# 0Setsuna0/SoftbodyUnity

Measured on AMD Instinct MI355X. Metric: particle-substeps/sec, higher is better.
Workload: dtype f32

## Files before the change

softbodyunity_amd/csrc/schedule.hip:

```cpp
#include "solver_internal.hpp"
#include "tile_kernel.hip.hpp"
#include "aux_kernels.hip.hpp"

namespace sbi {

sbk::TickParams tick_params(const sb_solver *s, float dt, int substeps) {
    sbk::TickParams t{};
    volatile float S = (float)substeps;
    volatile float h = dt / S;
    t.h = h;
    volatile float inv_h = 1.0f / h;
    t.inv_h = inv_h;
    volatile float hx = h * s->desc.gravity[0], hy = h * s->desc.gravity[1], hz = h * s->desc.gravity[2];
    t.hgx = hx; t.hgy = hy; t.hgz = hz;
    volatile float td = s->desc.damping * h;
    volatile float kd = 1.0f - td;
    t.kd = kd < 0.0f ? 0.0f : (float)kd;
    volatile float h2 = h * h;
    volatile float ad = s->compliance[0] / h2;
    volatile float av = s->compliance[1] / h2;
    volatile float av36 = 36.0f * av;
    volatile float ab = s->compliance[2] / h2;
    t.at_d = ad; t.at_v = av36; t.at_b = ab;
    t.pnx = s->plane[0]; t.pny = s->plane[1]; t.pnz = s->plane[2]; t.pd = s->plane[3]; t.plane_on = s->plane_on;
// ... 112 lines not shown
        int cs = D.send_off[k + 1] - D.send_off[k], cr = D.recv_off[k + 1] - D.recv_off[k];
        if (s->loopback) cs = cr = std::min(cs, cr);
        const size_t fl = with_prev ? 6 : 3;
        if (cs) NCCL_CHECK(rccl().Send(s->d_sendbuf.p + fl * D.send_off[k], fl * (size_t)cs, ncclFloat, s->loopback ? 0 : D.peers[k], s->comm, st));
        if (cr) NCCL_CHECK(rccl().Recv(s->d_recvbuf.p + fl * D.recv_off[k], fl * (size_t)cr, ncclFloat, s->loopback ? 0 : D.peers[k], s->comm, st));
    }
}

void halo_exchange_post(sb_solver *s, int slot, hipStream_t st) {
    if (!halo_slot_active(s, slot) || s->peer.enabled) return;
    DevHalo &D = *s->halos[slot];
    const bool with_prev = slot == 1;
    const int nr = D.recv_off.back();
    if (nr && !(with_prev && s->fused_unpack)) {
        if (with_prev)
            hipLaunchKernelGGL(sbk::halo_unpack_kernel<true>, dim3((nr + 255) / 256), dim3(256), 0, st, s->pos_view(),
                               s->d_prev.p, D.recv_idx.p, s->d_recvbuf.p, nr);
        else
            hipLaunchKernelGGL(sbk::halo_unpack_kernel<false>, dim3((nr + 255) / 256), dim3(256), 0, st, s->pos_view(),
                               s->d_prev.p, D.recv_idx.p, s->d_recvbuf.p, nr);
    }
}

void ExchangeTimer::mark(hipStream_t st, bool join) {
    Event e;
    if (free_list.empty()) e.create(); else { e = std::move(free_list.back()); free_list.pop_back(); }
    HIP_CHECK(hipEventRecord(e, st));
    (join ? join_pending : pending).push_back(std::move(e));
}
void ExchangeTimer::recycle() {
    for (auto *v : {&pending, &join_pending}) {
        free_list.insert(free_list.end(), std::make_move_iterator(v->begin()), std::make_move_iterator(v->end()));
        v->clear();
    }
}

void halo_exchange(sb_solver *s, int slot, hipStream_t st) {
    if (!st) st = s->stream;
    if (!halo_slot_active(s, slot)) return;
    const bool timed = s->xtimer.enabled && !s->capturing;
    if (timed) s->xtimer.mark(st);
    if (!s->peer.enabled) halo_exchange_pre(s, slot, st);
    if (timed) s->xtimer.mark(st);
    if (s->peer.enabled) halo_exchange_pre(s, slot, st);
    if (!s->peer.enabled) {
        NCCL_CHECK(rccl().GroupStart());
        try {
            halo_exchange_calls(s, slot, st);
        } catch (...) {
            (void)rccl().GroupEnd();
            throw;
        }
        NCCL_CHECK(rccl().GroupEnd());
    }
    halo_exchange_post(s, slot, st);
    if (timed) s->xtimer.mark(st);
}

template <int KIND>
void launch_tile(sb_solver *s, DevTiling &D, int tile_begin = 0, int tile_end = -1, int halo = sbk::kHaloNone, const sbk::TileDesc *table = nullptr) {
    const bool ghosts = halo == sbk::kHaloGhosts;
    if (tile_end < 0) tile_end = D.n_tiles;
    if (tile_end <= tile_begin) return;
    sbk::TileArgs A{};
    A.pos = s->pos_view(); A.w8 = s->d_w8.p; A.wpal = s->d_wpal.p; A.prev = s->d_prev.p; A.vel = s->d_vel.p;
    A.tiles = D.tiles.p; A.runs_overflow = D.runs_overflow.p; A.stream = D.stream.p;
    A.tp = s->d_tp.p;
    A.gather = D.gather.p;
    A.w_uniform = s->w_uniform ? 1 : 0;
    A.item_waves = D.item_waves;
    A.store_through = tile_end - tile_begin <= s->store_through_max_tiles ? 3 : s->store_through_large;
    A.ghost_src = ghosts ? s->d_recvbuf.p : nullptr; A.n_owned = (int32_t)s->n_owned;
    A.peek_out = KIND == 4 ? s->d_peek.p : nullptr;
    A.kin_map = KIND == 5 ? s->d_kin_map.p : nullptr; A.kin_target = KIND == 5 ? s->d_kin_target.p : nullptr;
    A.max_local = D.max_local; A.win_dwords = D.win_dwords; A.tile_base = tile_begin; A.pal_dwords = D.pal_dwords; A.rounds_dwords = D.rounds_dwords;
    const sbk::TileDesc *tiles_at_base = table ? table : D.tiles.p + tile_begin;
    const int n_wg = tile_end - tile_begin;
    const bool small = D.max_local <= sbk::kSmallTile;
    const bool narrow = small && (D.packed_lanes ? D.packed_lanes == sbk::kLanePackLanes : (s->tile_lanes ? s->tile_lanes == sbk::kNarrowTileThreads : tile_end - tile_begin >= s->narrow_min_tiles));
    const bool quad8 = D.has_quads && s->quad_lanes == sbk::kQuadTileThreads;
    constexpr int kWide8MaxTiles = sbk::kWide8MaxTiles;
    const bool wide8 = small && !D.has_quads && !D.packed_lanes && (s->tile_lanes ? s->tile_lanes == 512 : tile_end - tile_begin <= kWide8MaxTiles);
    const dim3 grid(tile_end - tile_begin), block(quad8 || wide8 ? sbk::kQuadTileThreads : (narrow ? sbk::kNarrowTileThreads : sbk::kWideTileThreads));
#define SB_LAUNCH_TILE(Q, W, G)                                                                                               \
    do {                                                                                                                      \
        if (Q && quad8) {                                                                                                     \
            if (small) hipLaunchKernelGGL((sbk::tile_kernel<KIND, true, sbk::kQuadTileThreads, sbk::kSmallTile / sbk::kQuadTileThreads, W, sbk::kHaloNone>), \
                                          grid, block, D.lds_bytes + s->lds_pad, s->stream, tiles_at_base, n_wg, A);                                           \
            else hipLaunchKernelGGL((sbk::tile_kernel<KIND, true, sbk::kQuadTileThreads, sbk::kLargeTile / sbk::kQuadTileThreads, W, sbk::kHaloNone>), \
                                    grid, block, D.lds_bytes + s->lds_pad, s->stream, tiles_at_base, n_wg, A);                                                 \
        } else if (wide8) hipLaunchKernelGGL((sbk::tile_kernel<KIND, false, sbk::kQuadTileThreads, sbk::kSmallTile / sbk::kQuadTileThreads, W, G>), \
                                       grid, block, D.lds_bytes + s->lds_pad, s->stream, tiles_at_base, n_wg, A);                                              \
        else if (narrow) hipLaunchKernelGGL((sbk::tile_kernel<KIND, Q, sbk::kNarrowTileThreads, sbk::kSmallTile / sbk::kNarrowTileThreads, W, G>), \
                                       grid, block, D.lds_bytes + s->lds_pad, s->stream, tiles_at_base, n_wg, A);                                              \
        else if (small) hipLaunchKernelGGL((sbk::tile_kernel<KIND, Q, sbk::kWideTileThreads, sbk::kSmallTile / sbk::kWideTileThreads, W, G>), \
                                           grid, block, D.lds_bytes + s->lds_pad, s->stream, tiles_at_base, n_wg, A);                                          \
        else hipLaunchKernelGGL((sbk::tile_kernel<KIND, Q, sbk::kWideTileThreads, sbk::kLargeTile / sbk::kWideTileThreads, W, G>), \
                                grid, block, D.lds_bytes + s->lds_pad, s->stream, tiles_at_base, n_wg, A);                                                     \
    } while (0)
    constexpr bool kCanGhost = KIND == 1 || KIND == 2;
    if (ghosts && !(kCanGhost && !D.has_quads)) throw std::runtime_error("internal: ghost-reading tile kernel requested for a launch that has none");
    if (kCanGhost && ghosts) {
        if (s->w_palette) SB_LAUNCH_TILE(false, true, (kCanGhost ? sbk::kHaloGhosts : sbk::kHaloNone)); else SB_LAUNCH_TILE(false, false, (kCanGhost ? sbk::kHaloGhosts : sbk::kHaloNone));
    } else
    if (s->w_palette) { if (D.has_quads) SB_LAUNCH_TILE(true, true, sbk::kHaloNone); else SB_LAUNCH_TILE(false, true, sbk::kHaloNone); }
    else { if (D.has_quads) SB_LAUNCH_TILE(true, false, sbk::kHaloNone); else SB_LAUNCH_TILE(false, false, sbk::kHaloNone); }
#undef SB_LAUNCH_TILE
}

struct LaunchTimer {
    std::vector<Event> ev;
    std::vector<int> slot;
    hipStream_t stream;
    void begin(int which) {
        Event a, b;
        a.create(); b.create();
        HIP_CHECK(hipEventRecord(a, stream));
        ev.push_back(std::move(a)); ev.push_back(std::move(b)); slot.push_back(which);
    }
    void end() { HIP_CHECK(hipEventRecord(ev.back(), stream)); }
};

void launch_tick_kernel(sb_solver *s, int it, int substeps, LaunchTimer *lt, int tile_begin = 0, int tile_end = -1, bool kin = false) {
    const int tl = s->plan->plan.tiling ? (it & 1) : 0;
    DevTiling &D = s->tiling[tl];
    if (lt && D.n_tiles) lt->begin(it == 0 ? 2 + (int)s->gcolours.size() : (it == substeps ? 3 + (int)s->gcolours.size() : tl));
    const int halo_in = s->fused_unpack && tl == 1 ? sbk::kHaloGhosts : sbk::kHaloNone;
    if (it == 0) launch_tile<0>(s, D, tile_begin, tile_end);
    else if (it < substeps && kin) launch_tile<5>(s, D, tile_begin, tile_end);
    else if (it < substeps) launch_tile<1>(s, D, tile_begin, tile_end, halo_in);
    else launch_tile<2>(s, D, tile_begin, tile_end, halo_in);
    if (lt && D.n_tiles) lt->end();
}

void launch_t2_layer(sb_solver *s, int layer, LaunchTimer *lt, bool with_halo = true) {
    const auto rg = s->t2_layer_range[layer];
    if (with_halo) halo_exchange(s, 2 + (int)s->gcolours.size() + layer);
    if (rg.second <= rg.first) return;
    if (lt) lt->begin(4 + (int)s->gcolours.size());
    launch_tile<3>(s, s->tiling[2], rg.first, rg.second);
    if (lt) lt->end();
}

void launch_gcolour(sb_solver *s, int gc, LaunchTimer *lt) {
    DevGColour &G = *s->gcolours[gc];
    if (G.count == 0) return;
    if (lt) lt->begin(2 + gc);
    dim3 grid((G.count + 255) / 256);
    if (G.type == 0)
        hipLaunchKernelGGL(sbk::global_distance_kernel, grid, dim3(256), 0, s->stream, s->pos_view(), G.ij.p, G.rest.p, G.count,
                           s->d_tp.p);
    else
        hipLaunchKernelGGL(sbk::global_quad_kernel, grid, dim3(256), 0, s->stream, s->pos_view(), G.quad.p, G.rest2.p, G.count,
                           G.type, s->d_tp.p);
    if (lt) lt->end();
}

std::vector<TickStep> tick_program(const sb_solver *s, int substeps, bool fused_first, bool defer_last, bool kin) {
    std::vector<TickStep> P;
    const bool two = s->plan->plan.tiling;
    auto tile = [&](int it, TileRange rg, bool k = false) {
        const bool ff = it == 0 && fused_first;
        P.push_back(TickStep{StepKind::Tile, rg, k && ff, ff ? 2 : it, ff ? 4 : substeps, 0});
    };
    if (s->overlap_halo) {
        for (int it = 0; it <= substeps; ++it) {
            if (it == substeps && defer_last) break;
            if (it & 1) {
                tile(it, TileRange::T1Interior);
                P.push_back(TickStep{StepKind::JoinExchange, TileRange::All, false, it, substeps, 1});
                tile(it, TileRange::T1Boundary);
            } else {
                tile(it, TileRange::T0Boundary);
                if (it < substeps) P.push_back(TickStep{StepKind::ForkExchange, TileRange::All, false, it, substeps, 1});
                tile(it, TileRange::T0Interior);
            }
        }
        return P;
    }
    for (int it = 0; it <= substeps; ++it) {
        if (it == substeps && defer_last) break;
        if (two && (it & 1)) P.push_back(TickStep{StepKind::Exchange, TileRange::All, false, it, substeps, 1});
        tile(it, TileRange::All, kin);
        if (it == substeps) break;
        for (size_t ly = 0; ly < s->t2_layer_range.size(); ++ly) {
            P.push_back(TickStep{StepKind::Exchange, TileRange::All, false, it, substeps, 2 + (int)s->gcolours.size() + (int)ly});
            P.push_back(TickStep{StepKind::T2Layer, TileRange::All, false, it, substeps, (int)ly});
        }
        for (size_t gc = 0; gc < s->gcolours.size(); ++gc) {
// ... 404 lines not shown
```

softbodyunity_amd/csrc/tile_kernel.hip.hpp:

```cpp
#pragma once
#include "device_math.hip.hpp"

namespace sbk {

__device__ __forceinline__ void lds_barrier() { asm volatile("s_waitcnt lgkmcnt(0)\n\ts_barrier" ::: "memory"); }

template <bool QUADS, int THREADS> constexpr int kWavesPerSimd = QUADS ? (THREADS == 64 ? 3 : (THREADS == 512 ? 2 : 4)) : (THREADS == 256 ? 8 : (THREADS == 128 ? 6 : 4));
template <int KIND_, bool QUADS, int THREADS, int PPT, bool WPAL, int HALO = kHaloNone>
__global__ __launch_bounds__(THREADS, (kWavesPerSimd<QUADS, THREADS> - (KIND_ == 5 && !QUADS ? 1 : 0))) void tile_kernel(const TileDesc *tiles_at_base, int n_workgroups, TileArgs A) {
    constexpr int KIND = KIND_ == 5 ? 1 : KIND_;
    constexpr bool KIN = KIND_ == 5;
    constexpr bool GHOSTS = HALO == kHaloGhosts;
    constexpr int kTileThreads = THREADS;
    constexpr int kCPL = THREADS >= kRoundSlots ? 1 : kRoundSlots / THREADS;
    extern __shared__ uint4 lds_raw[];
    float4 *lds_pos = reinterpret_cast<float4 *>(lds_raw);
    uint32_t *s_rounds = reinterpret_cast<uint32_t *>(lds_pos + A.max_local);
    float *s_pal = reinterpret_cast<float *>(s_rounds + A.rounds_dwords);
    uint32_t *cbuf = s_rounds + A.rounds_dwords + A.pal_dwords;
    f32x3 *lds_spare = reinterpret_cast<f32x3 *>(cbuf + A.win_dwords);
    typedef const TileDesc __attribute__((address_space(4))) *ConstTileDescPtr;
#ifndef SB_NO_XCD_REMAP
    const int nwg = n_workgroups, wg = (int)blockIdx.x;
    const int xq = nwg >> 3, xr = nwg & 7, xcd = wg & 7;
    const int tile_index = (xcd < xr ? xcd * (xq + 1) : xr * (xq + 1) + (xcd - xr) * xq) + (wg >> 3);
#else
    const int tile_index = (int)blockIdx.x;
#endif
    const TileDesc __attribute__((address_space(4))) &td = *((ConstTileDescPtr)(uintptr_t)tiles_at_base + tile_index);
    const int n_rounds_all = td.n_rounds;
    const int tid = threadIdx.x;
    const int n_local = td.n_local;
    const int run_count = td.run_count;
    const TickParams tp = *A.tp;
    const uint32_t *tstream = A.stream + td.s_begin;
#if defined(SB_ABLATE) && SB_ABLATE == 4
    if (n_local >= 0) { if (n_rounds_all == 0x7fffffff) A.vel[0] = tp.h; return; }
#endif

    int g[PPT];
    if (KIND == 3) {
#pragma unroll
        for (int m = 0; m < PPT; ++m) {
            const int l = tid + m * kTileThreads;
            g[m] = l < n_local ? A.gather[td.gather_begin + l] : -1;
        }
    } else {
        int run_d[kInlineRuns], run_y[kInlineRuns];
#pragma unroll
        for (int r = 0; r < kInlineRuns; ++r) { run_y[r] = td.runs[r].y; run_d[r] = td.runs[r].x - td.runs[r].y; }
#pragma unroll
        for (int m = 0; m < PPT; ++m) {
            const int l = tid + m * kTileThreads;
            int d = run_d[0];
#pragma unroll
            for (int r = 1; r < kInlineRuns; ++r) d = l >= run_y[r] ? run_d[r] : d;
            int gi = l + d;
            if (run_count > kInlineRuns)
                for (int r = kInlineRuns; r < run_count; ++r) {
                    const int2 rn = A.runs_overflow[td.run_overflow + r - kInlineRuns];
                    if (rn.y <= l) gi = rn.x + (l - rn.y);
                }
            g[m] = l < n_local ? gi : -1;
        }
    }
    const int R = n_rounds_all;
    const int v_begin = KIND == 0 ? R : 0;
    const int v_end = KIND == 3 ? R : (KIND == 2 || KIND == 4 ? R + 1 : 2 * R + 1);
    const uint32_t d_lo = td.s_hdr;
    const uint32_t d_hi = td.s_len;
    const uint32_t win = (uint32_t)A.win_dwords;
    uint32_t win_lo = d_lo;
    auto load_window = [&](uint32_t lo) {
        const uint32_t n4 = (min(lo + win, d_hi) - lo) >> 2;
        const uint4 *src = reinterpret_cast<const uint4 *>(tstream + lo);
        uint4 *dst = reinterpret_cast<uint4 *>(cbuf);
        uint32_t t0 = (uint32_t)tid;
        asm volatile("" : "+v"(t0));
        for (uint32_t i = t0; i < n4; i += 4 * kTileThreads) {
            uint4 v0 = src[i], v1, v2, v3;
            const bool b1 = i + kTileThreads < n4, b2 = i + 2 * kTileThreads < n4, b3 = i + 3 * kTileThreads < n4;
            if (b1) v1 = src[i + kTileThreads];
            if (b2) v2 = src[i + 2 * kTileThreads];
            if (b3) v3 = src[i + 3 * kTileThreads];
            dst[i] = v0;
            if (b1) dst[i + kTileThreads] = v1;
            if (b2) dst[i + 2 * kTileThreads] = v2;
            if (b3) dst[i + 3 * kTileThreads] = v3;
        }
    };
    f32x4 X[PPT];
    float pvx[PPT], pvy[PPT], pvz[PPT];
    uint32_t wi[PPT];
    const int mypal = WPAL ? __float_as_int(A.wpal[tid & (kMaxMassPalette - 1)]) : 0;
#pragma unroll
    for (int m = 0; m < PPT; ++m) {
        const int gc = max(g[m], 0);
        const bool ghost = GHOSTS && gc >= A.n_owned;
        const float *px = ghost ? A.ghost_src + 6 * (size_t)(gc - A.n_owned) : A.pos.xyz + 3 * (size_t)gc;
        X[m].x = px[0]; X[m].y = px[1]; X[m].z = px[2];
        if (WPAL) { wi[m] = A.w8[A.w_uniform ? 0 : gc]; X[m].w = 0.0f; } else { wi[m] = 0; X[m].w = A.pos.w[gc]; }
        pvx[m] = pvy[m] = pvz[m] = 0.0f;
        if (KIND != 0 && KIND != 3 && KIND != 4) {
            const float *pp = ghost ? px + 3 : A.prev + 3 * (size_t)gc;
            pvx[m] = pp[0]; pvy[m] = pp[1]; pvz[m] = pp[2];
        }
    }
    const bool rounds_in_lds = n_rounds_all <= A.rounds_dwords;
    const uint32_t rw = tstream[max(min(tid, n_rounds_all - 1), 0)];
    const bool rounds_in_lanes = n_rounds_all <= 64;
    const uint32_t rwl = tstream[max(min(tid & 63, n_rounds_all - 1), 0)];
    uint32_t itreg = 0;
    if (QUADS && kTileThreads == 64 * A.item_waves) {
        const int ns = td.n_steps;
        itreg = tstream[ns > 0 ? td.s_items + (uint32_t)((tid >> 6) * ns + min(tid & 63, ns - 1)) : 0u];
    }
    const int n_pal = td.n_pal;
    const uint32_t palw = tstream[tid < n_pal ? ((n_rounds_all + 3) & ~3) + tid : 0];
#ifndef SB_KW
#define SB_KW (QUADS ? 4 : 2)
#endif
    constexpr int kW = SB_KW;
    const bool lane_packed = !QUADS && kTileThreads == kLanePackLanes && td.packed_lanes == (uint32_t)kLanePackLanes;
    const bool lane_packed_full = !WPAL && lane_packed && td.n_pal == 0;
    const bool wide_packed = !QUADS && kTileThreads == kWidePackLanes && td.packed_lanes == (uint32_t)kWidePackLanes;
    const bool any_packed = lane_packed || wide_packed;
    const uint32_t n4_first = wide_packed ? 0u : lane_packed ? (lane_packed_full ? 2u * (uint32_t)kLanePackLanes : (uint32_t)kLanePackLanes)
                                          : (min(win_lo + win, d_hi) - win_lo) >> 2;
    const u32x4 *wsrc = reinterpret_cast<const u32x4 *>(tstream + win_lo);
    u32x4 wv[kW];
#pragma unroll
    for (int q = 0; q < kW; ++q) {
        const uint32_t i = tid + q * kTileThreads;
        wv[q] = i < n4_first ? wsrc[i] : *reinterpret_cast<const u32x4 *>(tstream);
    }
    typedef uint32_t u32x2 __attribute__((ext_vector_type(2)));
    u32x2 wc = {0u, 0u};
    u32x2 wp = {0u, 0u};
    if (!QUADS && kTileThreads == kWidePackLanes)
        wp = *reinterpret_cast<const u32x2 *>(wide_packed ? tstream + win_lo + 2u * (uint32_t)tid : tstream);
#pragma unroll
    for (int m = 0; m < PPT; ++m) asm volatile("" ::"v"(X[m].x), "v"(pvx[m]), "v"(wi[m]), "v"(X[m].w));
    asm volatile("" ::"v"(mypal));
    if (WPAL) {
#pragma unroll
        for (int m = 0; m < PPT; ++m) X[m].w = __int_as_float(__builtin_amdgcn_ds_bpermute((int)(wi[m] << 2), mypal));
    }
#pragma unroll
    for (int q = 0; q < kW; ++q) asm volatile("" ::"v"(wv[q].x));
    asm volatile("" ::"v"(rw), "v"(palw), "v"(rwl), "v"(itreg));
    if (!QUADS && kTileThreads == kWidePackLanes) asm volatile("" ::"v"(wp.x));
#pragma unroll
    for (int m = 0; m < PPT; ++m)
        if (g[m] >= 0) *reinterpret_cast<f32x4 *>(lds_pos + tid + m * kTileThreads) = X[m];
    if (rounds_in_lds && tid < n_rounds_all) s_rounds[tid] = rw;
    if (tid < n_pal) s_pal[tid] = __uint_as_float(palw);
    if (kTileThreads < kMaxRoundsLds && rounds_in_lds)
        for (int q = tid + kTileThreads; q < n_rounds_all; q += kTileThreads) s_rounds[q] = tstream[q];
    if (kTileThreads < kMaxPalette)
        for (int q = tid + kTileThreads; q < n_pal; q += kTileThreads) s_pal[q] = __uint_as_float(tstream[((n_rounds_all + 3) & ~3) + q]);
    {
        u32x4 *dst = reinterpret_cast<u32x4 *>(cbuf);
#pragma unroll
        for (int q = 0; q < kW; ++q) {
            const uint32_t i = tid + q * kTileThreads;
            if (i < n4_first && !any_packed) dst[i] = wv[q];
        }
        if (!any_packed)
            for (uint32_t i = tid + kW * kTileThreads; i < n4_first; i += kTileThreads) dst[i] = wsrc[i];
    }
    __syncthreads();
    if (!WPAL && !QUADS && kTileThreads == kLanePackLanes && lane_packed_full)
        wc = *reinterpret_cast<const u32x2 *>(tstream + win_lo + 8u * (uint32_t)kLanePackLanes + 2u * (uint32_t)tid);
#if defined(SB_ABLATE) && SB_ABLATE == 5
    if (n_local >= 0) { if (lds_pos[tid].x == 1.2345e-30f && cbuf[tid] == 0x12345678u) A.vel[0] = tp.h; return; }
#endif

    auto mark_step = [&]() {
#pragma unroll
        for (int m = 0; m < PPT; ++m)
            if (g[m] >= 0) {
                const int l = tid + m * kTileThreads;
                float4 P = lds_pos[l];
                if (KIND != 0 && tp.plane_on && P.w > 0.0f) {
                    float a = tp.pnx * P.x, b = tp.pny * P.y, c = tp.pnz * P.z;
                    float pen = ((a + b) + c) - tp.pd;
                    if (pen < 0.0f) {
                        float dx = pen * tp.pnx, dy = pen * tp.pny, dz = pen * tp.pnz;
                        P.x = P.x - dx; P.y = P.y - dy; P.z = P.z - dz;
                        if (KIND == 2 || KIND == 4) lds_pos[l] = P;
                    }
                }
                if (KIND == 4) continue;
                float vx, vy, vz;
                const size_t o = 3 * (size_t)g[m];
                if (KIND == 0) {
                    vx = A.vel[o + 0]; vy = A.vel[o + 1]; vz = A.vel[o + 2];
                } else {
                    float dx = P.x - pvx[m], dy = P.y - pvy[m], dz = P.z - pvz[m];
                    float qx = dx * tp.inv_h, qy = dy * tp.inv_h, qz = dz * tp.inv_h;
                    vx = qx * tp.kd; vy = qy * tp.kd; vz = qz * tp.kd;
                }
                bool moved = false;
                if (KIN && P.w == 0.0f) {
                    const int ks = A.kin_map[g[m]];
                    if (ks >= 0) {
                        float *t = A.kin_target + 3 * (size_t)ks;
                        const float tx = t[0], ty = t[1], tz = t[2];
                        if (tx == tx) { P.x = tx; P.y = ty; P.z = tz; moved = true; t[0] = __int_as_float(0x7fc00000); }
                    }
                }
                if (KIND == 2) {
                    A.vel[o + 0] = vx; A.vel[o + 1] = vy; A.vel[o + 2] = vz;
                } else {
                    if (A.store_through & 1) store3_through(A.prev + o, P.x, P.y, P.z);
                    else { A.prev[o + 0] = P.x; A.prev[o + 1] = P.y; A.prev[o + 2] = P.z; }
                    if (P.w > 0.0f) {
                        vx = vx + tp.hgx; vy = vy + tp.hgy; vz = vz + tp.hgz;
                        float hx = tp.h * vx, hy = tp.h * vy, hz = tp.h * vz;
                        P.x = P.x + hx; P.y = P.y + hy; P.z = P.z + hz;
                        lds_pos[l] = P;
                    } else if (KIN && moved) lds_pos[l] = P;
                }
            }
    };

    constexpr int kRegRounds = THREADS >= 256 ? kRegRoundsWide : kRegRoundsNarrow;
    if (kRegRounds > 0 && !QUADS && n_rounds_all <= kRegRounds && n_rounds_all > 0 && (kRegFullSlots || n_pal > 0) && (any_packed || d_hi - d_lo <= win)) {
        const bool tile_compact = n_pal > 0;
        uint32_t rs[kRegRounds > 0 ? kRegRounds : 1][kCPL];
        float rl[kRegRounds > 0 ? kRegRounds : 1][kCPL];
        int rcnt[kRegRounds > 0 ? kRegRounds : 1];
        {
            uint32_t o = 0;
#pragma unroll
            for (int r = 0; r < kRegRounds; ++r) {
                rcnt[r] = 0;
                if (r < n_rounds_all) {
                    rcnt[r] = (int)((uint32_t)__builtin_amdgcn_readlane((int)rwl, r) & 1023u);
                    if (kCPL == 2 && lane_packed) {
#pragma unroll
                        for (int u = 0; u < kCPL; ++u) {
                            const int bit = kLanePackFieldBits * (2 * r + u), w0 = bit >> 5, sh = bit & 31;
                            const uint32_t lo = wv[0][w0] >> sh;
                            const uint32_t hi = (sh + kLanePackFieldBits > 32) ? (wv[0][w0 + 1 < 4 ? w0 + 1 : 3] << ((32 - sh) & 31)) : 0u;
                            const uint32_t f = (lo | hi) & ((1u << kLanePackFieldBits) - 1u);
                            rs[r][u] = (f & 511u) | (((f >> 9) & 511u) << 12) | ((f >> 18) << 24);
                            if (!WPAL) {
                                const int fld = 2 * r + u;
                                rl[r][u] = __uint_as_float(fld < 4 ? wv[1][fld < 4 ? fld : 0] : wc[fld >= 4 ? fld - 4 : 0]);
                            }
                        }
                    } else if (kCPL == 1 && wide_packed) {
                        const uint64_t two = (uint64_t)wp.x | ((uint64_t)wp.y << 32);
                        const uint32_t f = (uint32_t)(two >> (kLanePackFieldBits * (r < kLanePackRounds ? r : 0))) & ((1u << kLanePackFieldBits) - 1u);
                        rs[r][0] = (f & 511u) | (((f >> 9) & 511u) << 12) | ((f >> 18) << 24);
                    } else if (tile_compact) {
#pragma unroll
                        for (int u = 0; u < kCPL; ++u) {
                            const int c = tid + u * kTileThreads;
                            rs[r][u] = cbuf[o + (c < rcnt[r] ? c : 0)];
                        }
                        o += ((uint32_t)rcnt[r] + 3u) & ~3u;
                    } else {
#pragma unroll
                        for (int u = 0; u < kCPL; ++u) {
                            const int c = tid + u * kTileThreads;
                            const uint2 e = *reinterpret_cast<const uint2 *>(cbuf + o + 2 * (c < rcnt[r] ? c : 0));
                            rs[r][u] = (e.x & 0xfffu) | ((e.x >> 16) << 12);
                            rl[r][u] = __uint_as_float(e.y);
                        }
                        o += (2u * (uint32_t)rcnt[r] + 3u) & ~3u;
                    }
                } else {
#pragma unroll
                    for (int u = 0; u < kCPL; ++u) { rs[r][u] = 0; rl[r][u] = 0.0f; }
                }
            }
            if (tile_compact) {
#pragma unroll
                for (int r = 0; r < kRegRounds; ++r)
#pragma unroll
                    for (int u = 0; u < kCPL; ++u) rl[r][u] = s_pal[rs[r][u] >> 24];
            }
        }
        auto reg_round = [&](const uint32_t (&e)[kCPL], const float (&L0)[kCPL], int cnt) {
            if (kCPL == 1) {
                if (tid < cnt) {
                    const int i = e[0] & 0xfffu, k = (e[0] >> 12) & 0xfffu;
                    float4 a = lds_pos[i], b = lds_pos[k];
                    if (project_distance(a, b, L0[0], tp.at_d)) { lds_pos[i] = a; lds_pos[k] = b; }
                }
            } else {
                int ci[kCPL], ck[kCPL];
                bool con[kCPL];
                f32x4 ca[kCPL], cb[kCPL];
#pragma unroll
                for (int u = 0; u < kCPL; ++u) {
                    con[u] = tid + u * kTileThreads < cnt;
                    ci[u] = e[u] & 0xfffu; ck[u] = (e[u] >> 12) & 0xfffu;
                    ca[u] = *reinterpret_cast<const f32x4 *>(lds_pos + ci[u]);
                    cb[u] = *reinterpret_cast<const f32x4 *>(lds_pos + ck[u]);
                }
#pragma unroll
                for (int u = 0; u < kCPL; ++u) {
                    float4 a = make_float4(ca[u].x, ca[u].y, ca[u].z, ca[u].w), b = make_float4(cb[u].x, cb[u].y, cb[u].z, cb[u].w);
                    con[u] = project_distance_nobranch(a, b, L0[u], tp.at_d) && con[u];
                    ca[u].x = a.x; ca[u].y = a.y; ca[u].z = a.z; cb[u].x = b.x; cb[u].y = b.y; cb[u].z = b.z;
                }
#pragma unroll
                for (int u = 0; u < kCPL; ++u) {
                    f32x3 *da = con[u] ? reinterpret_cast<f32x3 *>(lds_pos + ci[u]) : lds_spare;
                    f32x3 *db = con[u] ? reinterpret_cast<f32x3 *>(lds_pos + ck[u]) : lds_spare;
                    *da = (f32x3){ca[u].x, ca[u].y, ca[u].z};
                    *db = (f32x3){cb[u].x, cb[u].y, cb[u].z};
                }
            }
            lds_barrier();
        };
#if defined(SB_ABLATE) && SB_ABLATE == 1
        constexpr bool kRunRounds = false;
#else
        constexpr bool kRunRounds = true;
#endif
        if (KIND != 0 && kRunRounds) {
#pragma unroll
            for (int r = 0; r < kRegRounds; ++r) if (r < n_rounds_all) reg_round(rs[r], rl[r], rcnt[r]);
        }
        if (KIND != 3) { mark_step(); lds_barrier(); }
        if ((KIND == 0 || KIND == 1) && kRunRounds) {
#pragma unroll
            for (int r = 0; r < kRegRounds; ++r) if (r < n_rounds_all) reg_round(rs[r], rl[r], rcnt[r]);
        }
    } else if (QUADS && kTileThreads == 64 * A.item_waves && td.n_steps > 0 && d_hi - d_lo <= win) {
        const int n_steps = td.n_steps;
        const int wave = __builtin_amdgcn_readfirstlane(tid >> 6), lane = tid & 63;
        const uint32_t *items = tstream + td.s_items + (uint32_t)(wave * n_steps);
        float *lds_f = reinterpret_cast<float *>(lds_pos);
        const int q = tid & 3;
        auto run_pass = [&]() {
            if (n_steps > 64) itreg = items[min(lane, n_steps - 1)];
#if defined(SB_ABLATE) && SB_ABLATE == 1
            if (n_steps >= 0) return;
#endif
#pragma unroll 1
            for (int st = 0; st < n_steps; ++st) {
                if ((st & 63) == 0 && st > 0) itreg = items[min(st + lane, n_steps - 1)];
                const uint32_t it = (uint32_t)__builtin_amdgcn_readlane((int)itreg, st & 63);
                const uint32_t type = it & 7u;
                const int cnt = (int)((it >> kItemCountShift) & 127u);
                const uint32_t *slots = cbuf + (it >> kItemOffsetShift);
                if (type == kItemBending) {
                    const int c = lane >> 4;
                    if (c < cnt) {
                        const uint4 e = *reinterpret_cast<const uint4 *>(slots + 4 * c);
                        const int k = (lane >> 2) & 3;
                        const int o0 = 4 * (int)(e.x & 0xffffu) + q, o1 = 4 * (int)(e.x >> 16) + q;
                        const int o2 = 4 * (int)(e.y & 0xffffu) + q, o3 = 4 * (int)(e.y >> 16) + q;
                        const float P[4] = {lds_f[o0], lds_f[o1], lds_f[o2], lds_f[o3]};
                        float Xk = k == 0 ? P[0] : (k == 1 ? P[1] : (k == 2 ? P[2] : P[3]));
                        const int ok_off = k == 0 ? o0 : (k == 1 ? o1 : (k == 2 ? o2 : o3));
#if defined(SB_ABLATE) && SB_ABLATE == 2
                        const bool ok = true; Xk += __uint_as_float(e.z) * P[1];
#else
                        const bool ok = project_bending_row(P, __uint_as_float(e.z), __uint_as_float(e.w), tp.at_b, k, (lane & 48) << 2, Xk);
#endif
                        if (ok && q < 3) lds_f[ok_off] = Xk;
                    }
                } else if (type == kItemVolume) {
                    const int c = lane >> 2;
                    if (c < cnt) {
                        const uint4 e = *reinterpret_cast<const uint4 *>(slots + 4 * c);
                        const int o0 = 4 * (int)(e.x & 0xffffu) + q, o1 = 4 * (int)(e.x >> 16) + q;
                        const int o2 = 4 * (int)(e.y & 0xffffu) + q, o3 = 4 * (int)(e.y >> 16) + q;
                        float P[4] = {lds_f[o0], lds_f[o1], lds_f[o2], lds_f[o3]};
#if defined(SB_ABLATE) && SB_ABLATE == 2
                        const bool ok = true; P[0] += __uint_as_float(e.z); P[1] -= P[2]; P[3] += P[0];
#else
                        const bool ok = project_volume_quad(P, __uint_as_float(e.z), tp.at_v);
#endif
                        if (ok && q < 3) { lds_f[o0] = P[0]; lds_f[o1] = P[1]; lds_f[o2] = P[2]; lds_f[o3] = P[3]; }
                    }
                } else if (type != kItemIdle) {
                    if (lane < cnt) {
                        int i, k;
                        float L0;
                        if (type == kItemDistCompact) {
                            const uint32_t e = slots[lane];
                            i = e & 0xfffu; k = (e >> 12) & 0xfffu; L0 = s_pal[e >> 24];
                        } else {
                            const uint2 e = *reinterpret_cast<const uint2 *>(slots + 2 * lane);
                            i = e.x & 0xffffu; k = e.x >> 16; L0 = __uint_as_float(e.y);
                        }
                        float4 a = lds_pos[i], b = lds_pos[k];
#if defined(SB_ABLATE) && SB_ABLATE == 2
                        a.x += L0; b.x -= tp.at_d; lds_pos[i] = a; lds_pos[k] = b;
#else
                        if (project_distance(a, b, L0, tp.at_d)) { lds_pos[i] = a; lds_pos[k] = b; }
// ... 4 lines not shown
            }
        };
        if (KIND != 0) run_pass();
        if (KIND != 3) { mark_step(); lds_barrier(); }
        if (KIND == 0 || KIND == 1) run_pass();
    } else {
    uint32_t off = d_lo;
#if defined(SB_ABLATE) && SB_ABLATE == 1
    for (int v = v_begin; v < v_end; v += 100000) {
#else
    for (int v = v_begin; v < v_end; ++v) {
#endif
        if (v == R) { mark_step(); lds_barrier(); continue; }
        const int r = v < R ? v : v - R - 1;
        if (v == R + 1) off = d_lo;
        uint32_t w;
        if (rounds_in_lanes) w = (uint32_t)__builtin_amdgcn_readlane((int)rwl, __builtin_amdgcn_readfirstlane(r));
        else if (rounds_in_lds) w = (uint32_t)__builtin_amdgcn_readfirstlane((int)s_rounds[r]);
        else w = (uint32_t)__builtin_amdgcn_readfirstlane((int)tstream[r]);
        const int cnt = w & 1023u, n_vol = (w >> 10) & 1023u, n_bend = (w >> 20) & 1023u;
        const bool compact = (w >> 30) & 1u;
        const uint32_t dsize = compact ? ((cnt + 3u) & ~3u) : ((2u * cnt + 3u) & ~3u);
        const uint32_t size = dsize + 4u * (uint32_t)(n_vol + n_bend);
        if (off + size > win_lo + win || off < win_lo) {
            lds_barrier();
            win_lo = off;
            load_window(win_lo);
            __syncthreads();
        }
        const uint32_t *base = cbuf + (off - win_lo);
        if (QUADS) {
            const int wave = __builtin_amdgcn_readfirstlane(tid >> 6), lane = tid & 63;
            const int n_wb = (n_bend + 15) >> 4, n_wv = (n_vol + 15) >> 4, n_wd = (cnt + 63) >> 6;
            const uint32_t *qbase = base + dsize;
            float *lds_f = reinterpret_cast<float *>(lds_pos);
            const int q = tid & 3;
            constexpr int kWavesPerTile = kTileThreads / 64;
            const int n_slots = n_wb + n_wv + n_wd;
#pragma unroll 1
            for (int row = 0; row * kWavesPerTile < n_slots; ++row) {
                const int sw = row * kWavesPerTile + ((row & 1) ? kWavesPerTile - 1 - wave : wave);
                if (sw >= n_slots) continue;
                if (sw < n_wb + n_wv) {
                    const bool bend = sw < n_wb;
                    const int c = (bend ? sw : sw - n_wb) * 16 + (lane >> 2);
                    if (c < (bend ? n_bend : n_vol)) {
                        const uint4 e = *reinterpret_cast<const uint4 *>(qbase + 4 * (bend ? n_vol + c : c));
                        const int o0 = 4 * (int)(e.x & 0xffffu) + q, o1 = 4 * (int)(e.x >> 16) + q;
                        const int o2 = 4 * (int)(e.y & 0xffffu) + q, o3 = 4 * (int)(e.y >> 16) + q;
                        float P[4] = {lds_f[o0], lds_f[o1], lds_f[o2], lds_f[o3]};
                        const bool ok = bend ? project_bending_quad(P, __uint_as_float(e.z), __uint_as_float(e.w), tp.at_b, q)
                                             : project_volume_quad(P, __uint_as_float(e.z), tp.at_v);
                        if (ok && q < 3) { lds_f[o0] = P[0]; lds_f[o1] = P[1]; lds_f[o2] = P[2]; lds_f[o3] = P[3]; }
                    }
                } else {
                    const int c = (sw - n_wb - n_wv) * 64 + lane;
                    if (c < cnt) {
                        int i, k;
                        float L0;
                        if (compact) {
                            const uint32_t e = base[c];
                            i = e & 0xfffu; k = (e >> 12) & 0xfffu; L0 = s_pal[e >> 24];
                        } else {
                            const uint2 e = *reinterpret_cast<const uint2 *>(base + 2 * c);
                            i = e.x & 0xffffu; k = e.x >> 16; L0 = __uint_as_float(e.y);
                        }
                        float4 a = lds_pos[i], b = lds_pos[k];
                        if (project_distance(a, b, L0, tp.at_d)) { lds_pos[i] = a; lds_pos[k] = b; }
                    }
                }
            }
        } else if (kCPL == 1) {
            if (tid < cnt) {
                int i, k;
                float L0;
                if (compact) {
                    const uint32_t e = base[tid];
                    i = e & 0xfffu; k = (e >> 12) & 0xfffu; L0 = s_pal[e >> 24];
                } else {
                    const uint2 e = *reinterpret_cast<const uint2 *>(base + 2 * tid);
                    i = e.x & 0xffffu; k = e.x >> 16; L0 = __uint_as_float(e.y);
                }
                float4 a = lds_pos[i], b = lds_pos[k];
#if defined(SB_ABLATE) && SB_ABLATE == 2
                a.x += L0; b.x -= tp.at_d;
                lds_pos[i] = a; lds_pos[k] = b;
#else
                if (project_distance(a, b, L0, tp.at_d)) { lds_pos[i] = a; lds_pos[k] = b; }
#endif
            }
        } else {
            int ci[kCPL], ck[kCPL];
            float cL0[kCPL];
            bool con[kCPL];
            f32x4 ca[kCPL], cb[kCPL];
            if (!compact) {
#pragma unroll
                for (int u = 0; u < kCPL; ++u) {
                    const int c = tid + u * kTileThreads;
                    con[u] = c < cnt;
                    const uint2 e = *reinterpret_cast<const uint2 *>(base + 2 * (con[u] ? c : 0));
                    ci[u] = e.x & 0xffffu; ck[u] = e.x >> 16; cL0[u] = __uint_as_float(e.y);
                }
            } else {
                uint32_t ce[kCPL];
#pragma unroll
                for (int u = 0; u < kCPL; ++u) {
                    const int c = tid + u * kTileThreads;
                    con[u] = c < cnt;
                    ce[u] = base[con[u] ? c : 0];
                }
#pragma unroll
                for (int u = 0; u < kCPL; ++u) { ci[u] = ce[u] & 0xfffu; ck[u] = (ce[u] >> 12) & 0xfffu; cL0[u] = s_pal[ce[u] >> 24]; }
            }
#pragma unroll
            for (int u = 0; u < kCPL; ++u) {
                ca[u] = *reinterpret_cast<const f32x4 *>(lds_pos + ci[u]);
                cb[u] = *reinterpret_cast<const f32x4 *>(lds_pos + ck[u]);
            }
#pragma unroll
            for (int u = 0; u < kCPL; ++u) {
                float4 a = make_float4(ca[u].x, ca[u].y, ca[u].z, ca[u].w), b = make_float4(cb[u].x, cb[u].y, cb[u].z, cb[u].w);
                con[u] = project_distance_nobranch(a, b, cL0[u], tp.at_d) && con[u];
                ca[u].x = a.x; ca[u].y = a.y; ca[u].z = a.z; cb[u].x = b.x; cb[u].y = b.y; cb[u].z = b.z;
            }
#pragma unroll
            for (int u = 0; u < kCPL; ++u) {
                f32x3 *da = con[u] ? reinterpret_cast<f32x3 *>(lds_pos + ci[u]) : lds_spare;
                f32x3 *db = con[u] ? reinterpret_cast<f32x3 *>(lds_pos + ck[u]) : lds_spare;
                *da = (f32x3){ca[u].x, ca[u].y, ca[u].z};
                *db = (f32x3){cb[u].x, cb[u].y, cb[u].z};
            }
        }
        off += size;
#if defined(SB_ABLATE) && SB_ABLATE == 3
        asm volatile("s_waitcnt lgkmcnt(0)" ::: "memory");
#else
        lds_barrier();
#endif
    }
    }
#pragma unroll
    for (int m = 0; m < PPT; ++m)
        if (g[m] >= 0) {
            const float4 P = lds_pos[tid + m * kTileThreads];
            if (KIND == 4) { float *o = A.peek_out + 3 * (size_t)g[m]; o[0] = P.x; o[1] = P.y; o[2] = P.z; }
            else if (A.store_through & 2) store3_through(A.pos.xyz + 3 * (size_t)g[m], P.x, P.y, P.z);
            else pv_store(A.pos, g[m], P);
        }
}


}
```

Measured before the change: 121.5 billion.

## Add uniform-mass tile kernel variant and precompute byte-offset constraint slots

```diff
diff --git a/softbodyunity_amd/csrc/schedule.hip b/softbodyunity_amd/csrc/schedule.hip
--- a/softbodyunity_amd/csrc/schedule.hip
+++ b/softbodyunity_amd/csrc/schedule.hip
@@ -218,7 +218,7 @@
     constexpr int kWide8MaxTiles = sbk::kWide8MaxTiles;
     const bool wide8 = small && !D.has_quads && !D.packed_lanes && (s->tile_lanes ? s->tile_lanes == 512 : tile_end - tile_begin <= kWide8MaxTiles);
     const dim3 grid(tile_end - tile_begin), block(quad8 || wide8 ? sbk::kQuadTileThreads : (narrow ? sbk::kNarrowTileThreads : sbk::kWideTileThreads));
-#define SB_LAUNCH_TILE(Q, W, G)                                                                                               \
+#define SB_LAUNCH_TILE(Q, W, G, O)                                                                                             \
     do {                                                                                                                      \
         if (Q && quad8) {                                                                                                     \
             if (small) hipLaunchKernelGGL((sbk::tile_kernel<KIND, true, sbk::kQuadTileThreads, sbk::kSmallTile / sbk::kQuadTileThreads, W, sbk::kHaloNone>), \
@@ -227,20 +227,23 @@
                                     grid, block, D.lds_bytes + s->lds_pad, s->stream, tiles_at_base, n_wg, A);                                                 \
         } else if (wide8) hipLaunchKernelGGL((sbk::tile_kernel<KIND, false, sbk::kQuadTileThreads, sbk::kSmallTile / sbk::kQuadTileThreads, W, G>), \
                                        grid, block, D.lds_bytes + s->lds_pad, s->stream, tiles_at_base, n_wg, A);                                              \
-        else if (narrow) hipLaunchKernelGGL((sbk::tile_kernel<KIND, Q, sbk::kNarrowTileThreads, sbk::kSmallTile / sbk::kNarrowTileThreads, W, G>), \
+        else if (narrow) hipLaunchKernelGGL((sbk::tile_kernel<KIND, Q, sbk::kNarrowTileThreads, sbk::kSmallTile / sbk::kNarrowTileThreads, W, G, O>), \
                                        grid, block, D.lds_bytes + s->lds_pad, s->stream, tiles_at_base, n_wg, A);                                              \
-        else if (small) hipLaunchKernelGGL((sbk::tile_kernel<KIND, Q, sbk::kWideTileThreads, sbk::kSmallTile / sbk::kWideTileThreads, W, G>), \
+        else if (small) hipLaunchKernelGGL((sbk::tile_kernel<KIND, Q, sbk::kWideTileThreads, sbk::kSmallTile / sbk::kWideTileThreads, W, G, O>), \
                                            grid, block, D.lds_bytes + s->lds_pad, s->stream, tiles_at_base, n_wg, A);                                          \
         else hipLaunchKernelGGL((sbk::tile_kernel<KIND, Q, sbk::kWideTileThreads, sbk::kLargeTile / sbk::kWideTileThreads, W, G>), \
                                 grid, block, D.lds_bytes + s->lds_pad, s->stream, tiles_at_base, n_wg, A);                                                     \
     } while (0)
     constexpr bool kCanGhost = KIND == 1 || KIND == 2;
     if (ghosts && !(kCanGhost && !D.has_quads)) throw std::runtime_error("internal: ghost-reading tile kernel requested for a launch that has none");
+    constexpr bool kCanOneW = KIND == 0 || KIND == 1 || KIND == 2 || KIND == 4;
+    const bool one_w = kCanOneW && s->w_uniform && s->w_palette && !D.has_quads && !ghosts && small && !wide8;
     if (kCanGhost && ghosts) {
-        if (s->w_palette) SB_LAUNCH_TILE(false, true, (kCanGhost ? sbk::kHaloGhosts : sbk::kHaloNone)); else SB_LAUNCH_TILE(false, false, (kCanGhost ? sbk::kHaloGhosts : sbk::kHaloNone));
+        if (s->w_palette) SB_LAUNCH_TILE(false, true, (kCanGhost ? sbk::kHaloGhosts : sbk::kHaloNone), false); else SB_LAUNCH_TILE(false, false, (kCanGhost ? sbk::kHaloGhosts : sbk::kHaloNone), false);
     } else
-    if (s->w_palette) { if (D.has_quads) SB_LAUNCH_TILE(true, true, sbk::kHaloNone); else SB_LAUNCH_TILE(false, true, sbk::kHaloNone); }
-    else { if (D.has_quads) SB_LAUNCH_TILE(true, false, sbk::kHaloNone); else SB_LAUNCH_TILE(false, false, sbk::kHaloNone); }
+    if (one_w) SB_LAUNCH_TILE(false, true, sbk::kHaloNone, kCanOneW);
+    else if (s->w_palette) { if (D.has_quads) SB_LAUNCH_TILE(true, true, sbk::kHaloNone, false); else SB_LAUNCH_TILE(false, true, sbk::kHaloNone, false); }
+    else { if (D.has_quads) SB_LAUNCH_TILE(true, false, sbk::kHaloNone, false); else SB_LAUNCH_TILE(false, false, sbk::kHaloNone, false); }
 #undef SB_LAUNCH_TILE
 }
 
diff --git a/softbodyunity_amd/csrc/tile_kernel.hip.hpp b/softbodyunity_amd/csrc/tile_kernel.hip.hpp
--- a/softbodyunity_amd/csrc/tile_kernel.hip.hpp
+++ b/softbodyunity_amd/csrc/tile_kernel.hip.hpp
@@ -6,7 +6,7 @@
 __device__ __forceinline__ void lds_barrier() { asm volatile("s_waitcnt lgkmcnt(0)\n\ts_barrier" ::: "memory"); }
 
 template <bool QUADS, int THREADS> constexpr int kWavesPerSimd = QUADS ? (THREADS == 64 ? 3 : (THREADS == 512 ? 2 : 4)) : (THREADS == 256 ? 8 : (THREADS == 128 ? 6 : 4));
-template <int KIND_, bool QUADS, int THREADS, int PPT, bool WPAL, int HALO = kHaloNone>
+template <int KIND_, bool QUADS, int THREADS, int PPT, bool WPAL, int HALO = kHaloNone, bool ONEW = false>
 __global__ __launch_bounds__(THREADS, (kWavesPerSimd<QUADS, THREADS> - (KIND_ == 5 && !QUADS ? 1 : 0))) void tile_kernel(const TileDesc *tiles_at_base, int n_workgroups, TileArgs A) {
     constexpr int KIND = KIND_ == 5 ? 1 : KIND_;
     constexpr bool KIN = KIND_ == 5;
@@ -38,6 +38,7 @@
     if (n_local >= 0) { if (n_rounds_all == 0x7fffffff) A.vel[0] = tp.h; return; }
 #endif
 
+    static_assert(!ONEW || (WPAL && !QUADS && HALO == kHaloNone && KIND_ != 3 && KIND_ != 5), "one-mass variant: spring kernels with palette masses only");
     int g[PPT];
     if (KIND == 3) {
 #pragma unroll
@@ -49,13 +50,36 @@
         int run_d[kInlineRuns], run_y[kInlineRuns];
 #pragma unroll
         for (int r = 0; r < kInlineRuns; ++r) { run_y[r] = td.runs[r].y; run_d[r] = td.runs[r].x - td.runs[r].y; }
+        int dl[PPT];
+#pragma unroll
+        for (int m = 0; m < PPT; ++m) dl[m] = run_d[0];
+        auto chain = [&](int r_lo, int r_hi) {
+#pragma unroll
+            for (int r = r_lo; r < r_hi; ++r)
+#pragma unroll
+                for (int m = 0; m < PPT; ++m) dl[m] = tid + m * kTileThreads >= run_y[r] ? run_d[r] : dl[m];
+        };
+        static_assert(kInlineRuns > 8, "the run chain is cut at 4 and 8");
+        if (kTileThreads >= 512) {
+#pragma unroll
+            for (int m = 0; m < PPT; ++m) {
+                const int l = tid + m * kTileThreads;
+                int d = run_d[0];
+#pragma unroll
+                for (int r = 1; r < kInlineRuns; ++r) d = l >= run_y[r] ? run_d[r] : d;
+                dl[m] = d;
+            }
+        } else if (run_count > 1) {
+            chain(1, 4);
+            if (run_count > 4) {
+                chain(4, 8);
+                if (run_count > 8) chain(8, kInlineRuns);
+            }
+        }
 #pragma unroll
         for (int m = 0; m < PPT; ++m) {
             const int l = tid + m * kTileThreads;
-            int d = run_d[0];
-#pragma unroll
-            for (int r = 1; r < kInlineRuns; ++r) d = l >= run_y[r] ? run_d[r] : d;
-            int gi = l + d;
+            int gi = l + dl[m];
             if (run_count > kInlineRuns)
                 for (int r = kInlineRuns; r < run_count; ++r) {
                     const int2 rn = A.runs_overflow[td.run_overflow + r - kInlineRuns];
@@ -93,13 +117,15 @@
     float pvx[PPT], pvy[PPT], pvz[PPT];
     uint32_t wi[PPT];
     const int mypal = WPAL ? __float_as_int(A.wpal[tid & (kMaxMassPalette - 1)]) : 0;
+    const uint32_t wi_one = ONEW ? A.w8[0] : 0u;
 #pragma unroll
     for (int m = 0; m < PPT; ++m) {
         const int gc = max(g[m], 0);
         const bool ghost = GHOSTS && gc >= A.n_owned;
         const float *px = ghost ? A.ghost_src + 6 * (size_t)(gc - A.n_owned) : A.pos.xyz + 3 * (size_t)gc;
         X[m].x = px[0]; X[m].y = px[1]; X[m].z = px[2];
-        if (WPAL) { wi[m] = A.w8[A.w_uniform ? 0 : gc]; X[m].w = 0.0f; } else { wi[m] = 0; X[m].w = A.pos.w[gc]; }
+        if (ONEW) { wi[m] = 0; X[m].w = 0.0f; }
+        else if (WPAL) { wi[m] = A.w8[A.w_uniform ? 0 : gc]; X[m].w = 0.0f; } else { wi[m] = 0; X[m].w = A.pos.w[gc]; }
         pvx[m] = pvy[m] = pvz[m] = 0.0f;
         if (KIND != 0 && KIND != 3 && KIND != 4) {
             const float *pp = ghost ? px + 3 : A.prev + 3 * (size_t)gc;
@@ -140,9 +166,16 @@
     if (!QUADS && kTileThreads == kWidePackLanes)
         wp = *reinterpret_cast<const u32x2 *>(wide_packed ? tstream + win_lo + 2u * (uint32_t)tid : tstream);
 #pragma unroll
-    for (int m = 0; m < PPT; ++m) asm volatile("" ::"v"(X[m].x), "v"(pvx[m]), "v"(wi[m]), "v"(X[m].w));
+    for (int m = 0; m < PPT; ++m) {
+        if (ONEW) asm volatile("" ::"v"(X[m].x), "v"(pvx[m]));
+        else asm volatile("" ::"v"(X[m].x), "v"(pvx[m]), "v"(wi[m]), "v"(X[m].w));
+    }
     asm volatile("" ::"v"(mypal));
-    if (WPAL) {
+    float w_one = 0.0f;
+    if (ONEW) {
+        asm volatile("" ::"v"(wi_one));
+        w_one = __int_as_float(__builtin_amdgcn_readlane(mypal, __builtin_amdgcn_readfirstlane((int)(wi_one & (kMaxMassPalette - 1)))));
+    } else if (WPAL) {
 #pragma unroll
         for (int m = 0; m < PPT; ++m) X[m].w = __int_as_float(__builtin_amdgcn_ds_bpermute((int)(wi[m] << 2), mypal));
     }
@@ -152,7 +185,10 @@
     if (!QUADS && kTileThreads == kWidePackLanes) asm volatile("" ::"v"(wp.x));
 #pragma unroll
     for (int m = 0; m < PPT; ++m)
-        if (g[m] >= 0) *reinterpret_cast<f32x4 *>(lds_pos + tid + m * kTileThreads) = X[m];
+        if (g[m] >= 0) {
+            if (ONEW) *reinterpret_cast<f32x3 *>(lds_pos + tid + m * kTileThreads) = (f32x3){X[m].x, X[m].y, X[m].z};
+            else *reinterpret_cast<f32x4 *>(lds_pos + tid + m * kTileThreads) = X[m];
+        }
     if (rounds_in_lds && tid < n_rounds_all) s_rounds[tid] = rw;
     if (tid < n_pal) s_pal[tid] = __uint_as_float(palw);
     if (kTileThreads < kMaxRoundsLds && rounds_in_lds)
@@ -176,19 +212,24 @@
     if (n_local >= 0) { if (lds_pos[tid].x == 1.2345e-30f && cbuf[tid] == 0x12345678u) A.vel[0] = tp.h; return; }
 #endif
 
+    auto lds_put = [&](int l, const float4 &P) {
+        if (ONEW) *reinterpret_cast<f32x3 *>(lds_pos + l) = (f32x3){P.x, P.y, P.z};
+        else lds_pos[l] = P;
+    };
     auto mark_step = [&]() {
 #pragma unroll
         for (int m = 0; m < PPT; ++m)
             if (g[m] >= 0) {
                 const int l = tid + m * kTileThreads;
                 float4 P = lds_pos[l];
+                if (ONEW) P.w = w_one;
                 if (KIND != 0 && tp.plane_on && P.w > 0.0f) {
                     float a = tp.pnx * P.x, b = tp.pny * P.y, c = tp.pnz * P.z;
                     float pen = ((a + b) + c) - tp.pd;
                     if (pen < 0.0f) {
                         float dx = pen * tp.pnx, dy = pen * tp.pny, dz = pen * tp.pnz;
                         P.x = P.x - dx; P.y = P.y - dy; P.z = P.z - dz;
-                        if (KIND == 2 || KIND == 4) lds_pos[l] = P;
+                        if (KIND == 2 || KIND == 4) lds_put(l, P);
                     }
                 }
                 if (KIND == 4) continue;
@@ -219,8 +260,8 @@
                         vx = vx + tp.hgx; vy = vy + tp.hgy; vz = vz + tp.hgz;
                         float hx = tp.h * vx, hy = tp.h * vy, hz = tp.h * vz;
                         P.x = P.x + hx; P.y = P.y + hy; P.z = P.z + hz;
-                        lds_pos[l] = P;
-                    } else if (KIN && moved) lds_pos[l] = P;
+                        lds_put(l, P);
+                    } else if (KIN && moved) lds_put(l, P);
                 }
             }
     };
@@ -228,9 +269,11 @@
     constexpr int kRegRounds = THREADS >= 256 ? kRegRoundsWide : kRegRoundsNarrow;
     if (kRegRounds > 0 && !QUADS && n_rounds_all <= kRegRounds && n_rounds_all > 0 && (kRegFullSlots || n_pal > 0) && (any_packed || d_hi - d_lo <= win)) {
         const bool tile_compact = n_pal > 0;
-        uint32_t rs[kRegRounds > 0 ? kRegRounds : 1][kCPL];
+        constexpr bool kByteSlots = THREADS < 512;
+        uint32_t rs[kRegRounds > 0 ? kRegRounds : 1][kCPL], rp[kRegRounds > 0 ? kRegRounds : 1][kCPL];
         float rl[kRegRounds > 0 ? kRegRounds : 1][kCPL];
         int rcnt[kRegRounds > 0 ? kRegRounds : 1];
+        auto slot_word = [](uint32_t i, uint32_t k, uint32_t pal) { return kByteSlots ? (i << 4) | (k << 20) : i | (k << 12) | (pal << 24); };
         {
             uint32_t o = 0;
 #pragma unroll
@@ -245,7 +288,7 @@
                             const uint32_t lo = wv[0][w0] >> sh;
                             const uint32_t hi = (sh + kLanePackFieldBits > 32) ? (wv[0][w0 + 1 < 4 ? w0 + 1 : 3] << ((32 - sh) & 31)) : 0u;
                             const uint32_t f = (lo | hi) & ((1u << kLanePackFieldBits) - 1u);
-                            rs[r][u] = (f & 511u) | (((f >> 9) & 511u) << 12) | ((f >> 18) << 24);
+                            rs[r][u] = slot_word(f & 511u, (f >> 9) & 511u, f >> 18); rp[r][u] = f >> 18;
                             if (!WPAL) {
                                 const int fld = 2 * r + u;
                                 rl[r][u] = __uint_as_float(fld < 4 ? wv[1][fld < 4 ? fld : 0] : wc[fld >= 4 ? fld - 4 : 0]);
@@ -254,12 +297,13 @@
                     } else if (kCPL == 1 && wide_packed) {
                         const uint64_t two = (uint64_t)wp.x | ((uint64_t)wp.y << 32);
                         const uint32_t f = (uint32_t)(two >> (kLanePackFieldBits * (r < kLanePackRounds ? r : 0))) & ((1u << kLanePackFieldBits) - 1u);
-                        rs[r][0] = (f & 511u) | (((f >> 9) & 511u) << 12) | ((f >> 18) << 24);
+                        rs[r][0] = slot_word(f & 511u, (f >> 9) & 511u, f >> 18); rp[r][0] = f >> 18;
                     } else if (tile_compact) {
 #pragma unroll
                         for (int u = 0; u < kCPL; ++u) {
                             const int c = tid + u * kTileThreads;
-                            rs[r][u] = cbuf[o + (c < rcnt[r] ? c : 0)];
+                            const uint32_t e = cbuf[o + (c < rcnt[r] ? c : 0)];
+                            rs[r][u] = kByteSlots ? slot_word(e & 0xfffu, (e >> 12) & 0xfffu, 0) : e; rp[r][u] = e >> 24;
                         }
                         o += ((uint32_t)rcnt[r] + 3u) & ~3u;
                     } else {
@@ -267,53 +311,68 @@
                         for (int u = 0; u < kCPL; ++u) {
                             const int c = tid + u * kTileThreads;
                             const uint2 e = *reinterpret_cast<const uint2 *>(cbuf + o + 2 * (c < rcnt[r] ? c : 0));
-                            rs[r][u] = (e.x & 0xfffu) | ((e.x >> 16) << 12);
+                            rs[r][u] = slot_word(e.x & 0xfffu, e.x >> 16, 0); rp[r][u] = 0;
                             rl[r][u] = __uint_as_float(e.y);
                         }
                         o += (2u * (uint32_t)rcnt[r] + 3u) & ~3u;
                     }
                 } else {
 #pragma unroll
-                    for (int u = 0; u < kCPL; ++u) { rs[r][u] = 0; rl[r][u] = 0.0f; }
+                    for (int u = 0; u < kCPL; ++u) { rs[r][u] = 0; rp[r][u] = 0; rl[r][u] = 0.0f; }
                 }
             }
             if (tile_compact) {
 #pragma unroll
                 for (int r = 0; r < kRegRounds; ++r)
 #pragma unroll
-                    for (int u = 0; u < kCPL; ++u) rl[r][u] = s_pal[rs[r][u] >> 24];
-            }
-        }
+                    for (int u = 0; u < kCPL; ++u) rl[r][u] = s_pal[kByteSlots ? rp[r][u] : rs[r][u] >> 24];
+            }
+        }
+        char *lds_bytes = reinterpret_cast<char *>(lds_pos);
         auto reg_round = [&](const uint32_t (&e)[kCPL], const float (&L0)[kCPL], int cnt) {
             if (kCPL == 1) {
                 if (tid < cnt) {
-                    const int i = e[0] & 0xfffu, k = (e[0] >> 12) & 0xfffu;
-                    float4 a = lds_pos[i], b = lds_pos[k];
-                    if (project_distance(a, b, L0[0], tp.at_d)) { lds_pos[i] = a; lds_pos[k] = b; }
+                    float4 *pa = kByteSlots ? reinterpret_cast<float4 *>(lds_bytes + (e[0] & 0xffffu)) : lds_pos + (e[0] & 0xfffu);
+                    float4 *pb = kByteSlots ? reinterpret_cast<float4 *>(lds_bytes + (e[0] >> 16)) : lds_pos + ((e[0] >> 12) & 0xfffu);
+                    float4 a = *pa, b = *pb;
+                    if (ONEW) { a.w = w_one; b.w = w_one; }
+                    if (project_distance(a, b, L0[0], tp.at_d)) {
+                        if (ONEW) {
+                            *reinterpret_cast<f32x3 *>(pa) = (f32x3){a.x, a.y, a.z}; *reinterpret_cast<f32x3 *>(pb) = (f32x3){b.x, b.y, b.z};
+                        } else { *pa = a; *pb = b; }
+                    }
                 }
             } else {
-                int ci[kCPL], ck[kCPL];
+                char *pi[kCPL], *pk[kCPL];
                 bool con[kCPL];
                 f32x4 ca[kCPL], cb[kCPL];
 #pragma unroll
                 for (int u = 0; u < kCPL; ++u) {
                     con[u] = tid + u * kTileThreads < cnt;
-                    ci[u] = e[u] & 0xfffu; ck[u] = (e[u] >> 12) & 0xfffu;
-                    ca[u] = *reinterpret_cast<const f32x4 *>(lds_pos + ci[u]);
-                    cb[u] = *reinterpret_cast<const f32x4 *>(lds_pos + ck[u]);
-                }
+                    pi[u] = lds_bytes + (e[u] & 0xffffu); pk[u] = lds_bytes + (e[u] >> 16);
+                    ca[u] = *reinterpret_cast<const f32x4 *>(pi[u]);
+                    cb[u] = *reinterpret_cast<const f32x4 *>(pk[u]);
+                }
+                bool all_stored = true;
 #pragma unroll
                 for (int u = 0; u < kCPL; ++u) {
-                    float4 a = make_float4(ca[u].x, ca[u].y, ca[u].z, ca[u].w), b = make_float4(cb[u].x, cb[u].y, cb[u].z, cb[u].w);
+                    float4 a = make_float4(ca[u].x, ca[u].y, ca[u].z, ONEW ? w_one : ca[u].w), b = make_float4(cb[u].x, cb[u].y, cb[u].z, ONEW ? w_one : cb[u].w);
                     con[u] = project_distance_nobranch(a, b, L0[u], tp.at_d) && con[u];
+                    all_stored = all_stored && con[u];
                     ca[u].x = a.x; ca[u].y = a.y; ca[u].z = a.z; cb[u].x = b.x; cb[u].y = b.y; cb[u].z = b.z;
                 }
-#pragma unroll
-                for (int u = 0; u < kCPL; ++u) {
-                    f32x3 *da = con[u] ? reinterpret_cast<f32x3 *>(lds_pos + ci[u]) : lds_spare;
-                    f32x3 *db = con[u] ? reinterpret_cast<f32x3 *>(lds_pos + ck[u]) : lds_spare;
-                    *da = (f32x3){ca[u].x, ca[u].y, ca[u].z};
-                    *db = (f32x3){cb[u].x, cb[u].y, cb[u].z};
+                if (__builtin_amdgcn_ballot_w64(!all_stored) == 0) {
+#pragma unroll
+                    for (int u = 0; u < kCPL; ++u) {
+                        *reinterpret_cast<f32x3 *>(pi[u]) = (f32x3){ca[u].x, ca[u].y, ca[u].z};
+                        *reinterpret_cast<f32x3 *>(pk[u]) = (f32x3){cb[u].x, cb[u].y, cb[u].z};
+                    }
+                } else {
+#pragma unroll
+                    for (int u = 0; u < kCPL; ++u) {
+                        *(con[u] ? reinterpret_cast<f32x3 *>(pi[u]) : lds_spare) = (f32x3){ca[u].x, ca[u].y, ca[u].z};
+                        *(con[u] ? reinterpret_cast<f32x3 *>(pk[u]) : lds_spare) = (f32x3){cb[u].x, cb[u].y, cb[u].z};
+                    }
                 }
             }
             lds_barrier();
@@ -484,11 +543,12 @@
                     i = e.x & 0xffffu; k = e.x >> 16; L0 = __uint_as_float(e.y);
                 }
                 float4 a = lds_pos[i], b = lds_pos[k];
+                if (ONEW) { a.w = w_one; b.w = w_one; }
 #if defined(SB_ABLATE) && SB_ABLATE == 2
                 a.x += L0; b.x -= tp.at_d;
                 lds_pos[i] = a; lds_pos[k] = b;
 #else
-                if (project_distance(a, b, L0, tp.at_d)) { lds_pos[i] = a; lds_pos[k] = b; }
+                if (project_distance(a, b, L0, tp.at_d)) { lds_put(i, a); lds_put(k, b); }
 #endif
             }
         } else {
@@ -522,7 +582,7 @@
             }
 #pragma unroll
             for (int u = 0; u < kCPL; ++u) {
-                float4 a = make_float4(ca[u].x, ca[u].y, ca[u].z, ca[u].w), b = make_float4(cb[u].x, cb[u].y, cb[u].z, cb[u].w);
+                float4 a = make_float4(ca[u].x, ca[u].y, ca[u].z, ONEW ? w_one : ca[u].w), b = make_float4(cb[u].x, cb[u].y, cb[u].z, ONEW ? w_one : cb[u].w);
                 con[u] = project_distance_nobranch(a, b, cL0[u], tp.at_d) && con[u];
                 ca[u].x = a.x; ca[u].y = a.y; ca[u].z = a.z; cb[u].x = b.x; cb[u].y = b.y; cb[u].z = b.z;
             }
```

Result: slower. 117.7 billion (-3.2%).
